# learner-shx/SVG-IR

Measured on AMD Instinct MI355X. Metric: Gaussian-surfels/sec fwd+bwd @800x800 (1 view), higher is better.
Workload: dtype f32; 1 GPU; cfg2: rgss path, P=200000 surfels, 800x800, SH degree 3, S=5, VS=0, fwd+bwd, one view per step per GPU (BASELINE.json configs[1] = cfg2 at N=1; configs[3] = cfg4, view r on rank r, at N>1); num_rendered=673008, parallelism=view-parallel x1, per_rank_cpus=not pinned

## Files before the change

### svg-ir_amd/csrc/binning.hip

```cpp
#include <algorithm>
#include <cassert>

#include "common.hpp"
#include "depth_sort_plan.hpp"

namespace svgir {

namespace {

constexpr int GS = 32;

__device__ __forceinline__ uint32_t key_top_fold(uint32_t a, uint32_t b) { return (a & b & 0xff00u) | ((a | b) & 0xffu); }

struct WeightArgs {
    const uint32_t* vals;
    uint32_t* wgtot;
    RadixWeights w;
};

template <int ITEMS, bool W = false, bool F = false>
__global__ void __launch_bounds__(BLOCK) radix_hist_kernel(const uint32_t* __restrict__ keys, int n_cap,
                                                           const uint32_t* __restrict__ n_dev, int bit_lo,
                                                           uint32_t mask, uint32_t* __restrict__ table,
                                                           uint32_t* __restrict__ gtot, WeightArgs wa) {
    __shared__ uint32_t hist[256];
    __shared__ uint32_t whist[W ? 256 : 1];
    const int n = n_dev ? (int)min((uint32_t)n_cap, n_dev[0]) : n_cap;
    hist[threadIdx.x] = 0;
    if constexpr (W) whist[threadIdx.x] = 0;
    __syncthreads();
    const int base = blockIdx.x * (BLOCK * ITEMS);
    uint32_t k[ITEMS];
#pragma unroll
    for (int i = 0; i < ITEMS; i++) k[i] = keys[max(0, min(base + i * BLOCK + (int)threadIdx.x, n - 1))];
    uint32_t w[W ? ITEMS : 1];
    if constexpr (W) {
        uint32_t g[ITEMS];
#pragma unroll
        for (int i = 0; i < ITEMS; i++) g[i] = wa.vals[max(0, min(base + i * BLOCK + (int)threadIdx.x, n - 1))];
#pragma unroll
        for (int i = 0; i < ITEMS; i++) w[i] = wa.w.tiles[2 * (size_t)g[i]];
    }
#pragma unroll
    for (int i = 0; i < ITEMS; i++) {
        const int e = base + i * BLOCK + threadIdx.x;
        if constexpr (F) { if (e < n && w[i] != 0u) atomicAdd(&hist[(k[i] >> bit_lo) & mask], 1u); }
        else if (e < n) atomicAdd(&hist[(k[i] >> bit_lo) & mask], 1u);
        if constexpr (W) if (e < n && w[i] != 0u) atomicAdd(&whist[(k[i] >> bit_lo) & mask], w[i]);
    }
    __syncthreads();
    const uint32_t c = hist[threadIdx.x];
    table[(size_t)blockIdx.x * 256 + threadIdx.x] = c;
    if (c) atomicAdd(&gtot[(size_t)(blockIdx.x / GS) * 256 + threadIdx.x], c);
    if constexpr (W) {
        const uint32_t wc = whist[threadIdx.x];
        if constexpr (!F) wa.w.wtable[(size_t)blockIdx.x * 256 + threadIdx.x] = wc;
        if (wc) atomicAdd(&wa.wgtot[(size_t)(blockIdx.x / GS) * 256 + threadIdx.x], wc);
    }
}

template <int ITEMS, bool W = false>
__global__ void __launch_bounds__(BLOCK) radix_scatter_kernel(const uint32_t* __restrict__ kin,
                                                              const uint32_t* __restrict__ vin,
                                                              uint32_t* __restrict__ kout, uint32_t* __restrict__ vout,
                                                              int n_cap, const uint32_t* __restrict__ n_dev, int bit_lo, int nbits,
                                                              const uint32_t* __restrict__ table,
                                                              const uint32_t* __restrict__ gtot, int ngroups, WeightArgs wa) {
    __shared__ uint32_t wcnt[4][256];
    __shared__ uint32_t wtot[4];
    __shared__ uint32_t wtot2[W ? 4 : 1], ksum[W ? 4 : 1], smax[W ? 4 : 1];
    const int t = threadIdx.x, lane = t & 63, wave = t >> 6;
    const uint32_t mask = (1u << nbits) - 1;
    const int n = n_dev ? (int)min((uint32_t)n_cap, n_dev[0]) : n_cap;
    const int base = blockIdx.x * (BLOCK * ITEMS) + wave * (64 * ITEMS);
    const unsigned long long lt_mask = (lane == 0) ? 0ull : (~0ull >> (64 - lane));
    uint32_t ks[ITEMS], vs[ITEMS], rk[ITEMS];
#pragma unroll
    for (int c = 0; c < ITEMS; c++) {
        const int e = base + c * 64 + lane;
        ks[c] = e < n ? kin[e] : 0u;
        vs[c] = e < n ? vin[e] : 0u;
    }
    uint32_t ws[W ? ITEMS : 1];
    if constexpr (W) {
#pragma unroll
        for (int c = 0; c < ITEMS; c++) ws[c] = base + c * 64 + lane < n ? wa.w.tiles[2 * (size_t)vs[c]] : 0u;
        if (blockIdx.x == 0) {
            uint32_t kv = 0xff00u;
#pragma unroll 8
            for (int j = t; j < wa.w.n_key_top; j += BLOCK) kv = key_top_fold(kv, wa.w.key_top[j]);
            kv = wave_reduce(kv, key_top_fold);
            if (lane == 0) ksum[wave] = kv;
        }
    }
#pragma unroll
    for (int w = 0; w < 4; w++) wcnt[w][t] = 0;
    uint32_t cursor;
    uint32_t wcursor = 0;
    {
        const int g = blockIdx.x / GS;
        uint32_t tot = 0, pre = 0, wsum = 0, wpre = 0;
#pragma unroll 8
        for (int gg = 0; gg < ngroups; gg++) {
            const uint32_t v = gtot[(size_t)gg * 256 + t];
            tot += v;
            pre += gg < g ? v : 0u;
            if constexpr (W) {
                const uint32_t wv = wa.wgtot[(size_t)gg * 256 + t];
                wsum += wv;
                wpre += gg < g ? wv : 0u;
            }
        }
#pragma unroll 8
        for (int b = g * GS; b < (int)blockIdx.x; b++) {
            pre += table[(size_t)b * 256 + t];
            if constexpr (W) wpre += wa.w.wtable[(size_t)b * 256 + t];
        }
        cursor = block_excl_scan<4>(tot, wtot) + pre;
        if constexpr (W) {
            uint32_t R;
            wcursor = block_excl_scan<4>(wsum, wtot2, &R) + wpre;
            if (blockIdx.x == 0 && t == 0) {
                const uint32_t summary = key_top_fold(key_top_fold(ksum[0], ksum[1]), key_top_fold(ksum[2], ksum[3]));
                wa.w.counters[0] = R;
                wa.w.counters[2] = summary;
                if (wa.w.host_out) {
                    const uint32_t viol = wa.w.violation ? (wa.w.violation[0] != 0u ? 1u : 0u) : 0u;
                    __hip_atomic_store(wa.w.host_out, ((unsigned long long)wa.w.host_tag << 32) | R, __ATOMIC_RELAXED, __HIP_MEMORY_SCOPE_SYSTEM);
                    __hip_atomic_store(wa.w.host_out + 1, ((unsigned long long)wa.w.host_tag << 32) | (viol << 16) | summary, __ATOMIC_RELAXED,
                                       __HIP_MEMORY_SCOPE_SYSTEM);
                }
            }
        }
    }
#pragma unroll
    for (int c = 0; c < ITEMS; c++) {
        const bool valid = base + c * 64 + lane < n;
        const uint32_t d = (ks[c] >> bit_lo) & mask;
        const unsigned long long same = wave_match(d, nbits, valid);
        const uint32_t in_round = (uint32_t)__popcll(same & lt_mask);
        const uint32_t prior = wcnt[wave][d];
        rk[c] = prior + in_round;
        if (valid && in_round == 0) wcnt[wave][d] = prior + (uint32_t)__popcll(same);
    }
    __syncthreads();
    if constexpr (W) {
        __shared__ uint32_t sV[BLOCK * ITEMS];
        __shared__ __attribute__((aligned(16))) uint32_t sS[BLOCK * ITEMS];
        __shared__ uint8_t sD[BLOCK * ITEMS];
        __shared__ uint32_t bstart[256], gcur[256], wgcur[256];
        const uint32_t c0 = wcnt[0][t], c1 = wcnt[1][t], c2 = wcnt[2][t], c3 = wcnt[3][t];
        const uint32_t bs = block_excl_scan<4>(c0 + c1 + c2 + c3, wtot);
        bstart[t] = bs; gcur[t] = cursor; wgcur[t] = wcursor;
        wcnt[0][t] = bs; wcnt[1][t] = bs + c0; wcnt[2][t] = bs + c0 + c1; wcnt[3][t] = bs + c0 + c1 + c2;
        __syncthreads();
        uint32_t span = 0;
#pragma unroll
        for (int c = 0; c < ITEMS; c++) {
            if (base + c * 64 + lane < n) {
                const uint32_t d = (ks[c] >> bit_lo) & mask;
                const uint32_t lp = wcnt[wave][d] + rk[c];
                sV[lp] = vs[c]; sS[lp] = ws[c]; sD[lp] = (uint8_t)d;
                if (ws[c] != 0u) span = max(span, gcur[d] + (lp - bstart[d]) + 1u);
            }
        }
        span = wave_reduce_max(span);
        if (lane == 0) smax[wave] = span;
        __syncthreads();
        const int nblk = min(BLOCK * ITEMS, n - (int)blockIdx.x * (BLOCK * ITEMS));
        uint32_t wv[ITEMS], sum = 0;
#pragma unroll
        for (int c = 0; c < ITEMS; c += 4) {
            const uint4 q = reinterpret_cast<const uint4*>(sS)[(t * ITEMS + c) >> 2];
            wv[c] = q.x; wv[c + 1] = q.y; wv[c + 2] = q.z; wv[c + 3] = q.w;
        }
#pragma unroll
        for (int c = 0; c < ITEMS; c++) { wv[c] = t * ITEMS + c < nblk ? wv[c] : 0u; sum += wv[c]; }
        uint32_t run = block_excl_scan<4>(sum, wtot2);
#pragma unroll
        for (int c = 0; c < ITEMS; c += 4) {
            uint4 q;
            q.x = run; run += wv[c]; q.y = run; run += wv[c + 1]; q.z = run; run += wv[c + 2]; q.w = run; run += wv[c + 3];
            reinterpret_cast<uint4*>(sS)[(t * ITEMS + c) >> 2] = q;
        }
        if (t == 0) {
            const uint32_t m = max(max(smax[0], smax[1]), max(smax[2], smax[3]));
            if (m != 0u) atomicMax(wa.w.counters + 3, m);
        }
        __syncthreads();
#pragma unroll
        for (int c = 0; c < ITEMS; c++) {
            const int i = c * BLOCK + t;
            if (i < nblk) {
                const uint32_t d = sD[i], b = bstart[d];
                const uint32_t pos = gcur[d] + ((uint32_t)i - b);
                vout[pos] = sV[i];
                wa.w.offsets[pos] = wgcur[d] + (sS[i] - sS[b]);
            }
        }
        return;
    }
    if (ITEMS >= 16) {
        __shared__ uint32_t sK[BLOCK * (ITEMS >= 16 ? ITEMS : 1)], sV[BLOCK * (ITEMS >= 16 ? ITEMS : 1)];
        __shared__ uint32_t bstart[256], gcur[256];
        const uint32_t c0 = wcnt[0][t], c1 = wcnt[1][t], c2 = wcnt[2][t], c3 = wcnt[3][t];
        const uint32_t bc = c0 + c1 + c2 + c3;
        const uint32_t bs = block_excl_scan<4>(bc, wtot);
        bstart[t] = bs; gcur[t] = cursor;
        wcnt[0][t] = bs; wcnt[1][t] = bs + c0; wcnt[2][t] = bs + c0 + c1; wcnt[3][t] = bs + c0 + c1 + c2;
        __syncthreads();
#pragma unroll
        for (int c = 0; c < ITEMS; c++) {
            if (base + c * 64 + lane < n) {
                const uint32_t lp = wcnt[wave][(ks[c] >> bit_lo) & mask] + rk[c];
                sK[lp] = ks[c]; sV[lp] = vs[c];
            }
        }
        __syncthreads();
        const int nblk = min(BLOCK * ITEMS, n - (int)blockIdx.x * (BLOCK * ITEMS));
#pragma unroll
        for (int c = 0; c < ITEMS; c++) {
            const int i = c * BLOCK + t;
            if (i < nblk) {
                const uint32_t k = sK[i], d = (k >> bit_lo) & mask;
                const uint32_t pos = gcur[d] + ((uint32_t)i - bstart[d]);
                kout[pos] = k;
                vout[pos] = sV[i];
            }
        }
        return;
    }
    {
        const uint32_t c0 = wcnt[0][t], c1 = wcnt[1][t], c2 = wcnt[2][t];
        __syncthreads();
        wcnt[0][t] = cursor; wcnt[1][t] = cursor + c0; wcnt[2][t] = cursor + c0 + c1; wcnt[3][t] = cursor + c0 + c1 + c2;
    }
    __syncthreads();
#pragma unroll
    for (int c = 0; c < ITEMS; c++) {
        if (base + c * 64 + lane < n) {
            const uint32_t pos = wcnt[wave][(ks[c] >> bit_lo) & mask] + rk[c];
            kout[pos] = ks[c];
            vout[pos] = vs[c];
        }
    }
}


template <int ITEMS>
__global__ void __launch_bounds__(BLOCK) depth_bucket_scatter_kernel(const uint32_t* __restrict__ kin, const uint32_t* __restrict__ vin,
                                                                     uint32_t* __restrict__ kout, uint32_t* __restrict__ vout,
                                                                     uint32_t* __restrict__ wout, int n, int bit_lo,
                                                                     const uint32_t* __restrict__ table, const uint32_t* __restrict__ gtot,
                                                                     const uint32_t* __restrict__ wgtot, int ngroups, RadixWeights w) {
    __shared__ uint32_t wcnt[4][256];
    __shared__ uint32_t wtot[4], wtot2[4], wtot3[4], ksum[4], wcul[4];
    const int t = threadIdx.x, lane = t & 63, wave = t >> 6;
    const int base = blockIdx.x * (BLOCK * ITEMS) + wave * (64 * ITEMS);
    const unsigned long long lt_mask = (lane == 0) ? 0ull : (~0ull >> (64 - lane));
    uint32_t ks[ITEMS], vs[ITEMS], ws[ITEMS], rk[ITEMS];
#pragma unroll
    for (int c = 0; c < ITEMS; c++) {
        const int e = base + c * 64 + lane;
        ks[c] = e < n ? kin[e] : 0u;
        vs[c] = e < n ? vin[e] : 0u;
    }
#pragma unroll
    for (int c = 0; c < ITEMS; c++) ws[c] = base + c * 64 + lane < n ? w.tiles[2 * (size_t)vs[c]] : 0u;
    if (blockIdx.x == 0) {
        uint32_t kv = 0xff00u;
#pragma unroll 8
        for (int j = t; j < w.n_key_top; j += BLOCK) kv = key_top_fold(kv, w.key_top[j]);
        kv = wave_reduce(kv, key_top_fold);
        if (lane == 0) ksum[wave] = kv;
    }
#pragma unroll
    for (int q = 0; q < 4; q++) wcnt[q][t] = 0;
    uint32_t cursor, nvis, cull_base;
    {
        const int g = blockIdx.x / GS;
        uint32_t tot = 0, pre = 0, wsum = 0;
#pragma unroll 8
        for (int gg = 0; gg < ngroups; gg++) {
            const uint32_t v = gtot[(size_t)gg * 256 + t];
            tot += v;
            pre += gg < g ? v : 0u;
            if (blockIdx.x == 0) wsum += wgtot[(size_t)gg * 256 + t];
        }
#pragma unroll 8
        for (int b = g * GS; b < (int)blockIdx.x; b++) pre += table[(size_t)b * 256 + t];
        cursor = block_excl_scan<4>(tot, wtot, &nvis) + pre;
        cull_base = nvis + blockIdx.x * (BLOCK * ITEMS) - block_sum<4>(pre, wtot3);
        if (blockIdx.x == 0) {
            uint32_t R;
            (void)block_excl_scan<4>(wsum, wtot2, &R);
            if (t == 0) {
                const uint32_t summary = key_top_fold(key_top_fold(ksum[0], ksum[1]), key_top_fold(ksum[2], ksum[3]));
                w.counters[0] = R;
                w.counters[2] = summary;
                w.counters[3] = nvis;
                if (w.host_out) {
                    const uint32_t viol = w.violation ? (w.violation[0] != 0u ? 1u : 0u) : 0u;
                    __hip_atomic_store(w.host_out, ((unsigned long long)w.host_tag << 32) | R, __ATOMIC_RELAXED, __HIP_MEMORY_SCOPE_SYSTEM);
                    __hip_atomic_store(w.host_out + 1, ((unsigned long long)w.host_tag << 32) | (viol << 16) | summary, __ATOMIC_RELAXED,
                                       __HIP_MEMORY_SCOPE_SYSTEM);
                }
            }
        }
    }
    uint32_t ncul = 0;
#pragma unroll
    for (int c = 0; c < ITEMS; c++) {
        const bool valid = base + c * 64 + lane < n && ws[c] != 0u;
        const uint32_t d = (ks[c] >> bit_lo) & 255u;
        const unsigned long long same = wave_match(d, 8, valid);
        const uint32_t in_round = (uint32_t)__popcll(same & lt_mask);
        const uint32_t prior = wcnt[wave][d];
        rk[c] = prior + in_round;
        if (valid && in_round == 0) wcnt[wave][d] = prior + (uint32_t)__popcll(same);
        const unsigned long long culled = __ballot(base + c * 64 + lane < n && ws[c] == 0u);
        if (!valid) rk[c] = ncul + (uint32_t)__popcll(culled & lt_mask);
        ncul += (uint32_t)__popcll(culled);
    }
    if (lane == 0) wcul[wave] = ncul;
    __syncthreads();
    {
        const uint32_t c0 = wcnt[0][t], c1 = wcnt[1][t], c2 = wcnt[2][t];
        __syncthreads();
        wcnt[0][t] = cursor; wcnt[1][t] = cursor + c0; wcnt[2][t] = cursor + c0 + c1; wcnt[3][t] = cursor + c0 + c1 + c2;
    }
    __syncthreads();
    for (int q = 0; q < wave; q++) cull_base += wcul[q];
#pragma unroll
    for (int c = 0; c < ITEMS; c++) {
        if (base + c * 64 + lane >= n) continue;
        if (ws[c] != 0u) {
            const uint32_t pos = wcnt[wave][(ks[c] >> bit_lo) & 255u] + rk[c];
            kout[pos] = ks[c];
            vout[pos] = vs[c];
            wout[pos] = ws[c];
        } else {
            vout[cull_base + rk[c]] = vs[c];
        }
    }
}

constexpr int DB_THREADS = 1024, DB_WAVES = DB_THREADS / 64, DB_ROUNDS = DEPTH_BUCKET_CAP / DB_THREADS;

template <bool CARRY, class Get, class Put>
__device__ __forceinline__ void bucket_pass(int m, int shift, Get get, Put put, uint32_t (*wcnt)[256], uint32_t* cur, uint32_t* wsum) {
    const int t = threadIdx.x, lane = t & 63, wave = t >> 6;
    const unsigned long long lt_mask = (lane == 0) ? 0ull : (~0ull >> (64 - lane));
    for (int i = t; i < DB_WAVES * 256; i += DB_THREADS) (&wcnt[0][0])[i] = 0u;
    __syncthreads();
    const int per = ((m + DB_WAVES - 1) / DB_WAVES + 63) & ~63;
    const int base = wave * per;
    uint2 it[DB_ROUNDS];
    uint32_t rk[DB_ROUNDS];
#pragma unroll
    for (int r = 0; r < DB_ROUNDS; r++) {
        if (r * 64 < per) {
            const int i = base + r * 64 + lane;
            const bool valid = i < m;
            it[r] = valid ? get(i) : make_uint2(0u, 0u);
            const uint32_t d = (it[r].x >> shift) & 255u;
            const unsigned long long same = wave_match(d, 8, valid);
            const uint32_t in_round = (uint32_t)__popcll(same & lt_mask);
            const uint32_t prior = wcnt[wave][d];
            rk[r] = prior + in_round;
            if (valid && in_round == 0) wcnt[wave][d] = prior + (uint32_t)__popcll(same);
        }
    }
    __syncthreads();
    uint32_t c[DB_WAVES], total = 0;
#pragma unroll
    for (int q = 0; q < DB_WAVES; q++) { c[q] = t < 256 ? wcnt[q][t] : 0u; total += c[q]; }
    uint32_t run;
    if constexpr (CARRY) run = t < 256 ? cur[t] : 0u;
    else run = block_excl_scan<DB_WAVES>(total, wsum);
    if (t < 256) {
#pragma unroll
        for (int q = 0; q < DB_WAVES; q++) { wcnt[q][t] = run; run += c[q]; }
        if constexpr (CARRY) cur[t] = run;
    }
    __syncthreads();
#pragma unroll
    for (int r = 0; r < DB_ROUNDS; r++) {
        if (r * 64 < per) {
            const int i = base + r * 64 + lane;
            if (i < m) put(wcnt[wave][(it[r].x >> shift) & 255u] + rk[r], it[r]);
        }
    }
    __syncthreads();
}

__global__ void __launch_bounds__(DB_THREADS) depth_bucket_sort_kernel(uint32_t* key0, uint32_t* val0, uint32_t* key1, uint32_t* val1, uint32_t* offsets,
                                                                       const uint32_t* __restrict__ tiles, const uint32_t* __restrict__ gtot,
                                                                       const uint32_t* __restrict__ wgtot, int ngroups, int cap) {
    __shared__ uint32_t sA[DEPTH_BUCKET_CAP], sB[DEPTH_BUCKET_CAP], sI[DEPTH_BUCKET_CAP], sW[DEPTH_BUCKET_CAP];
    __shared__ uint32_t wcnt[DB_WAVES][256];
    __shared__ uint32_t cur[256], wsum[DB_WAVES], wsum2[DB_WAVES], hdr[3], red[2][DB_WAVES];
    const int t = threadIdx.x, lane = t & 63, wave = t >> 6;
    uint32_t cnt = 0, wt = 0;
    if (t < 256)
        for (int g = 0; g < ngroups; g++) { cnt += gtot[(size_t)g * 256 + t]; wt += wgtot[(size_t)g * 256 + t]; }
    const uint32_t cpre = block_excl_scan<DB_WAVES>(cnt, wsum);
    const uint32_t wpre = block_excl_scan<DB_WAVES>(wt, wsum2);
    if (t == (int)blockIdx.x) { hdr[0] = cpre; hdr[1] = cnt; hdr[2] = wpre; }
    __syncthreads();
    const uint32_t start = hdr[0], wbase = hdr[2];
    const int n = (int)hdr[1];
    if (n == 0) return;
    if (n <= cap) {
        for (int i = t; i < n; i += DB_THREADS) {
            sA[i] = (key1[start + i] << 16) | (uint32_t)i;
            sI[i] = val1[start + i];
            sW[i] = offsets[start + i];
        }
        bucket_pass<false>(n, 16, [&](int i) { return make_uint2(sA[i], 0u); }, [&](uint32_t pos, uint2 it) { sB[pos] = it.x; }, wcnt, cur, wsum);
        bucket_pass<false>(n, 24, [&](int i) { return make_uint2(sB[i], 0u); }, [&](uint32_t pos, uint2 it) { sA[pos] = it.x; }, wcnt, cur, wsum);
        uint32_t wv[DB_ROUNDS], sum = 0;
#pragma unroll
        for (int j = 0; j < DB_ROUNDS; j++) {
            const int i = t * DB_ROUNDS + j;
            wv[j] = i < n ? sW[sA[i] & 0xffffu] : 0u;
            sum += wv[j];
        }
        uint32_t run = block_excl_scan<DB_WAVES>(sum, wsum2);
#pragma unroll
        for (int j = 0; j < DB_ROUNDS; j++) {
            const int i = t * DB_ROUNDS + j;
            if (i < n) sB[i] = run;
            run += wv[j];
        }
        __syncthreads();
        for (int i = t; i < n; i += DB_THREADS) {
            val1[start + i] = sI[sA[i] & 0xffffu];
            offsets[start + i] = wbase + sB[i];
        }
        return;
    }
    {
        uint32_t a = 0xffffu, o = 0u;
        for (int i = t; i < n; i += DB_THREADS) { const uint32_t k = key1[start + i] & 0xffffu; a &= k; o |= k; }
        a = wave_reduce(a, [](uint32_t x, uint32_t y) { return x & y; });
        o = wave_reduce(o, [](uint32_t x, uint32_t y) { return x | y; });
        if (lane == 0) { red[0][wave] = a; red[1][wave] = o; }
        __syncthreads();
        a = 0xffffu; o = 0u;
#pragma unroll
        for (int q = 0; q < DB_WAVES; q++) { a &= red[0][q]; o |= red[1][q]; }
        if (a != o) {
            for (int pass = 0; pass < 2; pass++) {
                const uint32_t* sk = (pass ? key0 : key1) + start; const uint32_t* sv = (pass ? val0 : val1) + start;
                uint32_t* dk = (pass ? key1 : key0) + start; uint32_t* dv = (pass ? val1 : val0) + start;
                const int shift = 8 * pass;
                if (t < 256) cur[t] = 0u;
                __syncthreads();
                for (int i = t; i < n; i += DB_THREADS) atomicAdd(&cur[(sk[i] >> shift) & 255u], 1u);
                __syncthreads();
                const uint32_t ex = block_excl_scan<DB_WAVES>(t < 256 ? cur[t] : 0u, wsum);
                if (t < 256) cur[t] = ex;
                for (int c0 = 0; c0 < n; c0 += cap)
                    bucket_pass<true>(min(cap, n - c0), shift, [&](int i) { return make_uint2(sk[c0 + i], sv[c0 + i]); },
                                      [&](uint32_t pos, uint2 it) { dk[pos] = it.x; dv[pos] = it.y; }, wcnt, cur, wsum);
                __threadfence_block();
                __syncthreads();
            }
        }
    }
    uint32_t carry = wbase;
    for (int c0 = 0; c0 < n; c0 += DB_THREADS * DB_ROUNDS) {
        uint32_t wv[DB_ROUNDS], sum = 0;
#pragma unroll
        for (int j = 0; j < DB_ROUNDS; j++) {
            const int i = c0 + t * DB_ROUNDS + j;
            wv[j] = i < n ? tiles[2 * (size_t)val1[start + i]] : 0u;
            sum += wv[j];
        }
        uint32_t all;
        uint32_t run = carry + block_excl_scan<DB_WAVES>(sum, wsum, &all);
#pragma unroll
        for (int j = 0; j < DB_ROUNDS; j++) {
            const int i = c0 + t * DB_ROUNDS + j;
            if (i < n) offsets[start + i] = run;
            run += wv[j];
        }
        carry += all;
        __syncthreads();
    }
}

__global__ void __launch_bounds__(BLOCK) ts12_hist_kernel(const uint32_t* __restrict__ keys, int n_cap, const uint32_t* __restrict__ n_dev,
                                                          uint32_t* __restrict__ table, int nbins) {
    __shared__ uint32_t hist[TS12_BINS];
    const int n = n_dev ? (int)min((uint32_t)n_cap, n_dev[0]) : n_cap;
    const int t = threadIdx.x;
    for (int i = t; i < nbins; i += BLOCK) hist[i] = 0u;
    __syncthreads();
    const int base = blockIdx.x * TS12_KEYS;
    uint32_t k[TS12_KEYS / BLOCK];
#pragma unroll
    for (int i = 0; i < TS12_KEYS / BLOCK; i++) k[i] = keys[max(0, min(base + i * BLOCK + t, n - 1))];
#pragma unroll
    for (int i = 0; i < TS12_KEYS / BLOCK; i++)
        if (base + i * BLOCK + t < n) atomicAdd(&hist[k[i] & (TS12_BINS - 1)], 1u);
    __syncthreads();
    uint32_t* row = table + (size_t)blockIdx.x * nbins;
    for (int i = t; i < nbins; i += BLOCK) row[i] = hist[i];
}

__global__ void __launch_bounds__(BLOCK) ts12_colscan_kernel(uint32_t* __restrict__ table, int nb, uint32_t* __restrict__ totals, int nbins) {
    __shared__ uint32_t psum[16][17];
    const int col = threadIdx.x & 15, seg = threadIdx.x >> 4;
    const int d = blockIdx.x * 16 + col;
    const int rps = (nb + 15) / 16, r0 = min(nb, seg * rps), r1 = min(nb, r0 + rps);
    uint32_t* colp = table + d;
    uint32_t sum = 0;
    int r = r0;
    for (; r + 8 <= r1; r += 8) {
        uint32_t c[8];
#pragma unroll
        for (int j = 0; j < 8; j++) c[j] = colp[(size_t)(r + j) * nbins];
#pragma unroll
        for (int j = 0; j < 8; j++) sum += c[j];
    }
    for (; r < r1; r++) sum += colp[(size_t)r * nbins];
    psum[seg][col] = sum;
    __syncthreads();
    uint32_t run = 0, all = 0;
#pragma unroll
    for (int sg = 0; sg < 16; sg++) { const uint32_t v = psum[sg][col]; run += sg < seg ? v : 0u; all += v; }
    if (seg == 0) totals[d] = all;
    r = r0;
    for (; r + 8 <= r1; r += 8) {
        uint32_t c[8];
#pragma unroll
        for (int j = 0; j < 8; j++) c[j] = colp[(size_t)(r + j) * nbins];
#pragma unroll
        for (int j = 0; j < 8; j++) { colp[(size_t)(r + j) * nbins] = run; run += c[j]; }
    }
    for (; r < r1; r++) { const uint32_t c = colp[(size_t)r * nbins]; colp[(size_t)r * nbins] = run; run += c; }
}

__global__ void __launch_bounds__(BLOCK) ts12_scatter_kernel(const uint32_t* __restrict__ kin, const uint32_t* __restrict__ vin,
                                                             uint32_t* __restrict__ kout, uint32_t* __restrict__ vout, int n_cap,
                                                             const uint32_t* __restrict__ n_dev, const uint32_t* __restrict__ table,
                                                             const uint32_t* __restrict__ totals, uint32_t* __restrict__ ranges, int T, int nbins) {
    __shared__ uint32_t cur[TS12_BINS];
    __shared__ uint16_t wcnt[4][TS12_BINS];
    __shared__ uint32_t wtot[4];
    constexpr int PERMAX = TS12_BINS / BLOCK;
    constexpr int ROUNDS = TS12_KEYS / BLOCK;
    const int per = nbins / BLOCK;
    const int t = threadIdx.x, lane = t & 63, wave = t >> 6;
    const int n = n_dev ? (int)min((uint32_t)n_cap, n_dev[0]) : n_cap;
    const int base = blockIdx.x * TS12_KEYS + wave * (64 * ROUNDS);
    const unsigned long long lt_mask = (lane == 0) ? 0ull : (~0ull >> (64 - lane));
    uint32_t ks[ROUNDS], vs[ROUNDS];
    uint16_t rk[ROUNDS];
#pragma unroll
    for (int c = 0; c < ROUNDS; c++) {
        const int e = base + c * 64 + lane;
        ks[c] = e < n ? kin[e] : 0u;
        vs[c] = e < n ? vin[e] : 0u;
    }
    uint32_t tot[PERMAX], pre[PERMAX];
    {
        const uint32_t* tp = totals + t * per;
        const uint32_t* rp = table + (size_t)blockIdx.x * nbins + t * per;
#pragma unroll
        for (int j = 0; j < PERMAX; j++) { tot[j] = j < per ? tp[j] : 0u; pre[j] = j < per ? rp[j] : 0u; }
    }
    uint32_t sum = 0;
#pragma unroll
    for (int j = 0; j < PERMAX; j++) sum += tot[j];
#pragma unroll
    for (int w = 0; w < 4; w++)
        for (int i = t; i < nbins / 2; i += BLOCK) reinterpret_cast<uint32_t*>(&wcnt[w][0])[i] = 0u;
    uint32_t run = block_excl_scan<4>(sum, wtot);
#pragma unroll
    for (int j = 0; j < PERMAX; j++) {
        if (j < per) {
            const int tile = t * per + j;
            cur[tile] = run + pre[j];
            if (blockIdx.x == 0 && tile < T) {
                ranges[2 * tile] = tot[j] ? run : 0u;
                ranges[2 * tile + 1] = tot[j] ? run + tot[j] : 0u;
            }
            run += tot[j];
        }
    }
#pragma unroll
    for (int c = 0; c < ROUNDS; c++) {
        const bool valid = base + c * 64 + lane < n;
        const uint32_t d = ks[c] & (TS12_BINS - 1);
        const unsigned long long same = wave_match(d, 12, valid);
        const uint32_t in_round = (uint32_t)__popcll(same & lt_mask);
        const uint32_t prior = wcnt[wave][d];
        rk[c] = (uint16_t)(prior + in_round);
        if (valid && in_round == 0) wcnt[wave][d] = (uint16_t)(prior + (uint32_t)__popcll(same));
    }
    __syncthreads();
#pragma unroll
    for (int c = 0; c < ROUNDS; c++) {
        if (base + c * 64 + lane < n) {
            const uint32_t d = ks[c] & (TS12_BINS - 1);
            uint32_t pos = cur[d] + rk[c];
            if (wave > 0) pos += wcnt[0][d];
            if (wave > 1) pos += wcnt[1][d];
            if (wave > 2) pos += wcnt[2][d];
            kout[pos] = ks[c];
            vout[pos] = vs[c];
        }
    }
}

__global__ void __launch_bounds__(BLOCK) emit_kernel(int P, const uint32_t* __restrict__ order,
                                                     const uint32_t* __restrict__ tiles,
                                                     const uint32_t* __restrict__ offsets, float* __restrict__ rec,
                                                     const int32_t* __restrict__ radii, int gx, int gy,
                                                     uint32_t* __restrict__ tile_keys, uint32_t* __restrict__ vals,
                                                     uint32_t cap, uint32_t* __restrict__ ranges, int n_ranges,
                                                     uint32_t* __restrict__ seg_count, uint32_t* __restrict__ gtot,
                                                     int n_gtot, const uint32_t* __restrict__ span,
                                                     uint32_t* __restrict__ disp_ctr) {
    const int i = blockIdx.x * BLOCK + threadIdx.x;
    for (int j = i; j < n_ranges; j += gridDim.x * BLOCK) ranges[j] = 0u;
    for (int j = i; j < n_gtot; j += gridDim.x * BLOCK) gtot[j] = 0u;
    for (int j = i; j < DISP_CTR_WORDS; j += gridDim.x * BLOCK) disp_ctr[j] = 0u;
    if (i == 0) seg_count[0] = 0u;
    const int lane = threadIdx.x & 63;
    const uint32_t nvis = min((uint32_t)P, span[0]);
    if ((uint32_t)(i - lane) >= nvis) return;
    const bool valid = (uint32_t)i < nvis;
    const uint32_t g = valid ? order[i] : 0u;
    const uint32_t off = valid ? offsets[i] : 0u;
    const uint2 tr = valid ? reinterpret_cast<const uint2*>(tiles)[g] : make_uint2(0u, 0u);
    const uint32_t n = tr.x, rect = tr.y;
    if (n != 0u) {
        rec[(size_t)g * REC + R_IBASE] = __builtin_bit_cast(float, off);
        rec[(size_t)g * REC + R_RECT] = __builtin_bit_cast(float, rect);
    }
    const uint32_t incl = wave_incl_scan_u32(n);
    const uint32_t loc = incl - n;
    const uint32_t M = (uint32_t)__builtin_amdgcn_readlane((int)incl, 63);
    const uint32_t base = (uint32_t)__builtin_amdgcn_readfirstlane((int)(off - loc));
    for (uint32_t j0 = 0; j0 < M; j0 += 64u) {
        const uint32_t j = j0 + (uint32_t)lane;
        int lo = 0;
#pragma unroll
        for (int step = 32; step >= 1; step >>= 1) {
            const int mid = lo + step;
            const uint32_t v = (uint32_t)__builtin_amdgcn_ds_bpermute(mid << 2, (int)loc);
            lo = v <= j ? mid : lo;
        }
        const uint32_t t = j - (uint32_t)__builtin_amdgcn_ds_bpermute(lo << 2, (int)loc);
        const uint32_t go = (uint32_t)__builtin_amdgcn_ds_bpermute(lo << 2, (int)g);
        const uint32_t ro = (uint32_t)__builtin_amdgcn_ds_bpermute(lo << 2, (int)rect);
        const uint32_t w = max(ro >> 20, 1u), ty = t / w, tx = t - ty * w;
        const uint32_t pos = base + j;
        if (j < M && pos < cap) {
            tile_keys[pos] = (((ro >> 10) & 1023u) + ty) * (uint32_t)gx + ((ro & 1023u) + tx);
            vals[pos] = go;
        }
    }
}

__global__ void __launch_bounds__(BLOCK) ranges_kernel(int R_cap, const uint32_t* __restrict__ R_dev,
                                                       const uint32_t* __restrict__ tile_keys,
                                                       uint32_t* __restrict__ ranges) {
    const int i = blockIdx.x * BLOCK + threadIdx.x;
    const int R = R_dev ? (int)min((uint32_t)R_cap, R_dev[0]) : R_cap;
    if (i >= R) return;
    const uint32_t cur = tile_keys[i];
    if (i == 0) ranges[2 * cur] = 0;
    else {
        const uint32_t prev = tile_keys[i - 1];
        if (cur != prev) { ranges[2 * prev + 1] = (uint32_t)i; ranges[2 * cur] = (uint32_t)i; }
    }
    if (i == R - 1) ranges[2 * cur + 1] = (uint32_t)R;
}

__global__ void __launch_bounds__(1024) order_xcd_kernel(const uint32_t* __restrict__ counts, int n, uint32_t* __restrict__ order,
                                                         uint32_t* __restrict__ prefix, uint32_t* __restrict__ slot_prefix,
                                                         uint32_t* __restrict__ total, unsigned long long* __restrict__ host_total,
                                                         uint32_t host_tag, uint32_t cap_R, long long cap_slots, uint32_t magic, int gx,
                                                         int order_n) {
    __shared__ uint32_t hist[1024];
    __shared__ uint32_t wsum[16];
    __shared__ unsigned long long wsum2[16];
    __shared__ uint32_t wzero[16];
    const int t = threadIdx.x, lane = t & 63, wave = t >> 6;
    const uint32_t c = blockIdx.x;
    hist[t] = 0;
    auto both = [](uint32_t v) { return (unsigned long long)v | ((unsigned long long)seg_slots(v) << 32); };
    const int per = ((n + 7) / 8 + 1023) / 1024 * 1024;
    const int p0 = min(n, (int)c * per), p1 = min(n, p0 + per);
    __syncthreads();
    unsigned long long before = 0;
    uint32_t zeros = 0;
    for (int i = t; i < n; i += 1024) {
        const uint32_t len = counts[i];
        const int tile = i >> 2;
        if (xcd_of_tile(tile % gx, tile / gx) == c) atomicAdd(&hist[1023u - min(1023u, len)], 1u);
        if (i < p0) before += both(len);
        zeros += len == 0u ? 1u : 0u;
    }
    before = wave_reduce_add(before);
    zeros = wave_reduce_add(zeros);
    if (lane == 0) { wsum2[wave] = before; wzero[wave] = zeros; }
    __syncthreads();
    unsigned long long run = 0;
    uint32_t n_empty = 0;
#pragma unroll
    for (int w = 0; w < 16; w++) { run += wsum2[w]; n_empty += wzero[w]; }
    uint32_t n_mine;
    hist[t] = block_excl_scan<16>(hist[t], wsum, &n_mine);
    __syncthreads();
    for (int i0 = p0; i0 < p1; i0 += 1024) {
        const int i = i0 + t;
        const unsigned long long v = both(i < p1 ? counts[i] : 0u);
        const unsigned long long inc = (unsigned long long)wave_incl_scan_u32((uint32_t)v) | ((unsigned long long)wave_incl_scan_u32((uint32_t)(v >> 32)) << 32);
        __syncthreads();
        unsigned long long all;
        const unsigned long long ex = run + block_excl_scan<16>(v, inc, wsum2, &all);
        if (i < p1) {
            if (prefix) prefix[i] = (uint32_t)ex;
            if (slot_prefix) slot_prefix[i] = (uint32_t)(ex >> 32);
        }
        run += all;
    }
    if (c == 7 && t == 0) {
        if (total) {
            total[1] = (uint32_t)run; total[2] = (uint32_t)(run >> 32);
            total[3] = magic; total[4] = cap_R; total[5] = (uint32_t)(unsigned long long)cap_slots; total[6] = (uint32_t)((unsigned long long)cap_slots >> 32);
        }
        if (host_total) {
            __hip_atomic_store(host_total + 2, ((unsigned long long)host_tag << 32) | (unsigned long long)((uint32_t)n - n_empty), __ATOMIC_RELAXED, __HIP_MEMORY_SCOPE_SYSTEM);
            __hip_atomic_store(host_total, ((unsigned long long)host_tag << 32) | (run & 0xffffffffull), __ATOMIC_RELAXED, __HIP_MEMORY_SCOPE_SYSTEM);
            __hip_atomic_store(host_total + 1, ((unsigned long long)host_tag << 32) | (run >> 32), __ATOMIC_RELAXED, __HIP_MEMORY_SCOPE_SYSTEM);
        }
    }
    for (int i = t; i < n; i += 1024) {
        const int tile = i >> 2;
        if (xcd_of_tile(tile % gx, tile / gx) != c) continue;
        const uint32_t len = counts[i];
        order[8u * atomicAdd(&hist[1023u - min(1023u, len)], 1u) + c] = (uint32_t)i;
    }
    for (uint32_t j = n_mine + (uint32_t)t; 8u * j + c < (uint32_t)order_n; j += 1024u) order[8u * j + c] = ORDER_NONE;
}

}

void launch_order_desc(const uint32_t* counts, int n, uint32_t* order, uint32_t* prefix, uint32_t* slot_prefix, uint32_t* totals,
                       unsigned long long* host_totals, uint32_t host_tag, uint32_t cap_R, long long cap_slots, uint32_t magic, int gx, int order_n,
                       hipStream_t s) {
    hipLaunchKernelGGL(order_xcd_kernel, dim3(8), dim3(1024), 0, s, counts, n, order, prefix, slot_prefix, totals, host_totals,
                       host_tag, cap_R, cap_slots, magic, gx, order_n);
}

template <int ITEMS>
static void radix_sort_impl(uint32_t* const key[2], uint32_t* const val[2], int n, const uint32_t* n_dev, int total_bits,
                            int bits_per_pass, uint32_t* tbl, uint32_t* gtot, hipStream_t s, const RadixWeights* weights) {
    const int per = BLOCK * ITEMS;
    const int nb = (n + per - 1) / per;
    const int ng = (nb + GS - 1) / GS;
    const int passes = (total_bits + bits_per_pass - 1) / bits_per_pass;
    assert(!weights || (n_dev == nullptr && bits_per_pass <= 8 && passes <= RADIX_WGTOT_SLOT));
    for (int p = 0; p < passes; p++) {
        const int lo = p * bits_per_pass, nbits = std::min(bits_per_pass, total_bits - lo);
        uint32_t* gt = gtot + (size_t)p * ng * 256;
        if (weights && p == passes - 1) {
            const WeightArgs wa{val[p & 1], gtot + (size_t)RADIX_WGTOT_SLOT * ng * 256, *weights};
            hipLaunchKernelGGL((radix_hist_kernel<ITEMS, true>), dim3(nb), dim3(BLOCK), 0, s, key[p & 1], n, n_dev, lo,
                               (1u << nbits) - 1, tbl, gt, wa);
            hipLaunchKernelGGL((radix_scatter_kernel<ITEMS, true>), dim3(nb), dim3(BLOCK), 0, s, key[p & 1], val[p & 1],
                               key[(p + 1) & 1], val[(p + 1) & 1], n, n_dev, lo, nbits, tbl, gt, ng, wa);
            break;
        }
        hipLaunchKernelGGL((radix_hist_kernel<ITEMS>), dim3(nb), dim3(BLOCK), 0, s, key[p & 1], n, n_dev, lo,
                           (1u << nbits) - 1, tbl, gt, WeightArgs{});
        hipLaunchKernelGGL((radix_scatter_kernel<ITEMS>), dim3(nb), dim3(BLOCK), 0, s, key[p & 1], val[p & 1],
                           key[(p + 1) & 1], val[(p + 1) & 1], n, n_dev, lo, nbits, tbl, gt, ng, WeightArgs{});
    }
}

void launch_radix_sort(uint32_t* const key[2], uint32_t* const val[2], int n, const uint32_t* n_dev, int total_bits,
                       int bits_per_pass, uint32_t* table, hipStream_t s, const RadixWeights* weights) {
    if (n <= 0) return;
    uint32_t* gtot = radix_gtot(table, n);
    if (n <= (1 << 20)) radix_sort_impl<4>(key, val, n, n_dev, total_bits, bits_per_pass, table, gtot, s, weights);
    else radix_sort_impl<16>(key, val, n, n_dev, total_bits, bits_per_pass, table, gtot, s, weights);
}

void launch_depth_bucket_sort(uint32_t* const key[2], uint32_t* const val[2], int n, uint32_t* table, int cap, hipStream_t s, const RadixWeights& w) {
    if (n <= 0) return;
    constexpr int ITEMS = 4;
    assert(n <= DEPTH_BUCKET_MAX_P && cap >= DEPTH_BUCKET_CAP_MIN && cap <= DEPTH_BUCKET_CAP);
    const int nb = (n + BLOCK * ITEMS - 1) / (BLOCK * ITEMS), ng = (nb + GS - 1) / GS;
    uint32_t* gtot = radix_gtot(table, n);
    uint32_t* wgtot = gtot + (size_t)RADIX_WGTOT_SLOT * ng * 256;
    const WeightArgs wa{val[0], wgtot, w};
    hipLaunchKernelGGL((radix_hist_kernel<ITEMS, true, true>), dim3(nb), dim3(BLOCK), 0, s, key[0], n, (const uint32_t*)nullptr, 16, 255u, table, gtot, wa);
    hipLaunchKernelGGL((depth_bucket_scatter_kernel<ITEMS>), dim3(nb), dim3(BLOCK), 0, s, key[0], val[0], key[1], val[1], w.offsets, n, 16, table, gtot,
                       wgtot, ng, w);
    hipLaunchKernelGGL(depth_bucket_sort_kernel, dim3(256), dim3(DB_THREADS), 0, s, key[0], val[0], key[1], val[1], w.offsets, w.tiles, gtot, wgtot, ng, cap);
}

void launch_emit(int P, const uint32_t* order, const uint32_t* tiles, const uint32_t* offsets, float* rec,
                 const int32_t* radii, int gx, int gy, uint32_t* tile_keys, uint32_t* vals, int cap, uint32_t* ranges,
                 uint32_t* seg_count, uint32_t* sort_table, const uint32_t* span, uint32_t* disp_ctr, hipStream_t s) {
    hipLaunchKernelGGL(emit_kernel, dim3((P + BLOCK - 1) / BLOCK), dim3(BLOCK), 0, s, P, order, tiles, offsets, rec,
                       radii, gx, gy, tile_keys, vals, (uint32_t)cap, ranges, 2 * gx * gy + (gx * gy + 255) / 256 * SEG_BLOCK_STRIDE, seg_count,
                       radix_gtot(sort_table, cap), (int)radix_gtot_words(cap), span, disp_ctr);
}

void launch_tile_sort12(uint32_t* const key[2], uint32_t* const val[2], int n, const uint32_t* n_dev, uint32_t* table, uint32_t* ranges, int T,
                        hipStream_t s) {
    if (n <= 0) return;
    const int nb = (n + TS12_KEYS - 1) / TS12_KEYS;
    const int nbins = (T + BLOCK - 1) / BLOCK * BLOCK;
    uint32_t* totals = table + (size_t)nb * nbins;
    hipLaunchKernelGGL(ts12_hist_kernel, dim3(nb), dim3(BLOCK), 0, s, key[0], n, n_dev, table, nbins);
    hipLaunchKernelGGL(ts12_colscan_kernel, dim3(nbins / 16), dim3(BLOCK), 0, s, table, nb, totals, nbins);
    hipLaunchKernelGGL(ts12_scatter_kernel, dim3(nb), dim3(BLOCK), 0, s, key[0], val[0], key[1], val[1], n, n_dev, table, totals, ranges, T, nbins);
}

void launch_ranges(int R, const uint32_t* R_dev, const uint32_t* tile_keys, uint32_t* ranges, int T, hipStream_t s) {
    if (R > 0) hipLaunchKernelGGL(ranges_kernel, dim3((R + BLOCK - 1) / BLOCK), dim3(BLOCK), 0, s, R, R_dev, tile_keys, ranges);
}

}
```

Baseline: 620.2 million surfels/s.

## Widen tile-sort blocks, trim to device count, drop sorted-key writes

The 12-bit tile sort now runs hist and scatter with configurable 512-thread blocks handling 8 keys per thread. That shrinks the per-block histogram table and the column-scan work. Blocks beyond the device-side count now exit early, and colscan uses the real block count. The scatter no longer writes sorted keys, only values, which assumes downstream code needs only the ranges and values. The wider blocks use more shared memory and registers per block, and a missed consumer of the sorted keys would break.

```diff
diff --git a/svg-ir_amd/csrc/binning.hip b/svg-ir_amd/csrc/binning.hip
--- a/svg-ir_amd/csrc/binning.hip
+++ b/svg-ir_amd/csrc/binning.hip
@@ -491,27 +491,36 @@
     }
 }
 
-__global__ void __launch_bounds__(BLOCK) ts12_hist_kernel(const uint32_t* __restrict__ keys, int n_cap, const uint32_t* __restrict__ n_dev,
+#ifndef TS12_THREADS_V
+#define TS12_THREADS_V 512
+#endif
+constexpr int TS12T = TS12_THREADS_V, TS12W = TS12T / 64, TS12K = 8 * TS12T;
+static_assert(TS12K >= TS12_KEYS && TS12_BINS % TS12T == 0, "common.hpp tile12_table_words sizes the table for rows of TS12_KEYS keys");
+__host__ __device__ constexpr int ts12_blocks(int n) { return (n + TS12K - 1) / TS12K; }
+__global__ void __launch_bounds__(TS12T) ts12_hist_kernel(const uint32_t* __restrict__ keys, int n_cap, const uint32_t* __restrict__ n_dev,
                                                           uint32_t* __restrict__ table, int nbins) {
     __shared__ uint32_t hist[TS12_BINS];
     const int n = n_dev ? (int)min((uint32_t)n_cap, n_dev[0]) : n_cap;
+    if ((int)blockIdx.x >= ts12_blocks(n)) return;
     const int t = threadIdx.x;
-    for (int i = t; i < nbins; i += BLOCK) hist[i] = 0u;
-    __syncthreads();
-    const int base = blockIdx.x * TS12_KEYS;
-    uint32_t k[TS12_KEYS / BLOCK];
-#pragma unroll
-    for (int i = 0; i < TS12_KEYS / BLOCK; i++) k[i] = keys[max(0, min(base + i * BLOCK + t, n - 1))];
-#pragma unroll
-    for (int i = 0; i < TS12_KEYS / BLOCK; i++)
-        if (base + i * BLOCK + t < n) atomicAdd(&hist[k[i] & (TS12_BINS - 1)], 1u);
+    for (int i = t; i < nbins; i += TS12T) hist[i] = 0u;
+    __syncthreads();
+    const int base = blockIdx.x * TS12K;
+    uint32_t k[TS12K / TS12T];
+#pragma unroll
+    for (int i = 0; i < TS12K / TS12T; i++) k[i] = keys[max(0, min(base + i * TS12T + t, n - 1))];
+#pragma unroll
+    for (int i = 0; i < TS12K / TS12T; i++)
+        if (base + i * TS12T + t < n) atomicAdd(&hist[k[i] & (TS12_BINS - 1)], 1u);
     __syncthreads();
     uint32_t* row = table + (size_t)blockIdx.x * nbins;
-    for (int i = t; i < nbins; i += BLOCK) row[i] = hist[i];
-}
-
-__global__ void __launch_bounds__(BLOCK) ts12_colscan_kernel(uint32_t* __restrict__ table, int nb, uint32_t* __restrict__ totals, int nbins) {
+    for (int i = t; i < nbins; i += TS12T) row[i] = hist[i];
+}
+
+__global__ void __launch_bounds__(BLOCK) ts12_colscan_kernel(uint32_t* __restrict__ table, int nb_cap, int n_cap, const uint32_t* __restrict__ n_dev,
+                                                             uint32_t* __restrict__ totals, int nbins) {
     __shared__ uint32_t psum[16][17];
+    const int nb = n_dev ? (int)min((uint32_t)nb_cap, (uint32_t)ts12_blocks((int)min((uint32_t)n_cap, n_dev[0]))) : nb_cap;
     const int col = threadIdx.x & 15, seg = threadIdx.x >> 4;
     const int d = blockIdx.x * 16 + col;
     const int rps = (nb + 15) / 16, r0 = min(nb, seg * rps), r1 = min(nb, r0 + rps);
@@ -543,19 +552,20 @@
     for (; r < r1; r++) { const uint32_t c = colp[(size_t)r * nbins]; colp[(size_t)r * nbins] = run; run += c; }
 }
 
-__global__ void __launch_bounds__(BLOCK) ts12_scatter_kernel(const uint32_t* __restrict__ kin, const uint32_t* __restrict__ vin,
-                                                             uint32_t* __restrict__ kout, uint32_t* __restrict__ vout, int n_cap,
+__global__ void __launch_bounds__(TS12T) ts12_scatter_kernel(const uint32_t* __restrict__ kin, const uint32_t* __restrict__ vin,
+                                                             uint32_t* __restrict__ vout, int n_cap,
                                                              const uint32_t* __restrict__ n_dev, const uint32_t* __restrict__ table,
                                                              const uint32_t* __restrict__ totals, uint32_t* __restrict__ ranges, int T, int nbins) {
     __shared__ uint32_t cur[TS12_BINS];
-    __shared__ uint16_t wcnt[4][TS12_BINS];
-    __shared__ uint32_t wtot[4];
-    constexpr int PERMAX = TS12_BINS / BLOCK;
-    constexpr int ROUNDS = TS12_KEYS / BLOCK;
-    const int per = nbins / BLOCK;
+    __shared__ uint16_t wcnt[TS12W][TS12_BINS];
+    uint32_t* wtot = cur;
+    constexpr int PERMAX = TS12_BINS / TS12T;
+    constexpr int ROUNDS = TS12K / TS12T;
+    const int per = nbins / TS12T;
     const int t = threadIdx.x, lane = t & 63, wave = t >> 6;
     const int n = n_dev ? (int)min((uint32_t)n_cap, n_dev[0]) : n_cap;
-    const int base = blockIdx.x * TS12_KEYS + wave * (64 * ROUNDS);
+    if (blockIdx.x != 0 && (int)blockIdx.x >= ts12_blocks(n)) return;
+    const int base = blockIdx.x * TS12K + wave * (64 * ROUNDS);
     const unsigned long long lt_mask = (lane == 0) ? 0ull : (~0ull >> (64 - lane));
     uint32_t ks[ROUNDS], vs[ROUNDS];
     uint16_t rk[ROUNDS];
@@ -576,9 +586,10 @@
 #pragma unroll
     for (int j = 0; j < PERMAX; j++) sum += tot[j];
 #pragma unroll
-    for (int w = 0; w < 4; w++)
-        for (int i = t; i < nbins / 2; i += BLOCK) reinterpret_cast<uint32_t*>(&wcnt[w][0])[i] = 0u;
-    uint32_t run = block_excl_scan<4>(sum, wtot);
+    for (int w = 0; w < TS12W; w++)
+        for (int i = t; i < nbins / 2; i += TS12T) reinterpret_cast<uint32_t*>(&wcnt[w][0])[i] = 0u;
+    uint32_t run = block_excl_scan<TS12W>(sum, wtot);
+    __syncthreads();
 #pragma unroll
     for (int j = 0; j < PERMAX; j++) {
         if (j < per) {
@@ -607,10 +618,9 @@
         if (base + c * 64 + lane < n) {
             const uint32_t d = ks[c] & (TS12_BINS - 1);
             uint32_t pos = cur[d] + rk[c];
-            if (wave > 0) pos += wcnt[0][d];
-            if (wave > 1) pos += wcnt[1][d];
-            if (wave > 2) pos += wcnt[2][d];
-            kout[pos] = ks[c];
+#pragma unroll
+            for (int w = 0; w < TS12W - 1; w++)
+                if (wave > w) pos += wcnt[w][d];
             vout[pos] = vs[c];
         }
     }
@@ -819,12 +829,12 @@
 void launch_tile_sort12(uint32_t* const key[2], uint32_t* const val[2], int n, const uint32_t* n_dev, uint32_t* table, uint32_t* ranges, int T,
                         hipStream_t s) {
     if (n <= 0) return;
-    const int nb = (n + TS12_KEYS - 1) / TS12_KEYS;
-    const int nbins = (T + BLOCK - 1) / BLOCK * BLOCK;
+    const int nb = ts12_blocks(n);
+    const int nbins = (T + TS12T - 1) / TS12T * TS12T;
     uint32_t* totals = table + (size_t)nb * nbins;
-    hipLaunchKernelGGL(ts12_hist_kernel, dim3(nb), dim3(BLOCK), 0, s, key[0], n, n_dev, table, nbins);
-    hipLaunchKernelGGL(ts12_colscan_kernel, dim3(nbins / 16), dim3(BLOCK), 0, s, table, nb, totals, nbins);
-    hipLaunchKernelGGL(ts12_scatter_kernel, dim3(nb), dim3(BLOCK), 0, s, key[0], val[0], key[1], val[1], n, n_dev, table, totals, ranges, T, nbins);
+    hipLaunchKernelGGL(ts12_hist_kernel, dim3(nb), dim3(TS12T), 0, s, key[0], n, n_dev, table, nbins);
+    hipLaunchKernelGGL(ts12_colscan_kernel, dim3(nbins / 16), dim3(BLOCK), 0, s, table, nb, n, n_dev, totals, nbins);
+    hipLaunchKernelGGL(ts12_scatter_kernel, dim3(nb), dim3(TS12T), 0, s, key[0], val[0], val[1], n, n_dev, table, totals, ranges, T, nbins);
 }
 
 void launch_ranges(int R, const uint32_t* R_dev, const uint32_t* tile_keys, uint32_t* ranges, int T, hipStream_t s) {
```

Measured after the change: 631.5 million surfels/s, median of 6. 1.02x the previous value.
